# blitzcode/cpp-11-ray-trace-march-framework

Hardware: AMD Instinct MI355X
Metric: Msamples/s at 1920x1080x4spp Cornell-Box+killeroo (higher is better)
Workload: dtype f32; 1 GPU; scenes[1, 8]_1920x1080x4; width=1920, height=1080, spp=4, kernel=0, parallelism=tile-shard x1

## Files before the change

cpp-11-ray-trace-march-framework_amd/__init__.py:

```python
import ctypes
import os

import numpy as np

HERE = os.path.dirname(os.path.abspath(__file__))
KERNEL_SOURCES = ("csrc/rt_kernels.hip", "csrc/rt_walk.h", "csrc/rt_kparams.h", "csrc/rt_plan.hip",
                  "csrc/rt_scene.h", "csrc/rt_tracer.hip", "csrc/rt_grid_build.hip", "csrc/rt_device.h",
                  "csrc/rt_internal.h", "csrc/rt_box_words.h", "csrc/rt_fref_slots.h", "csrc/Makefile",
                  "../include/rt_tracer.h")


def kernel_source_hash():
    import hashlib
    h = hashlib.sha256()
    for rel in KERNEL_SOURCES:
        with open(os.path.normpath(os.path.join(HERE, rel)), "rb") as fh:
            h.update(fh.read())
    return h.hexdigest()[:16]
REPO = os.path.dirname(HERE)
SCENE_DIR = os.path.join(REPO, "data", "scenes")
MESH_DATA_DIR = os.path.join(REPO, "data", "meshes")

RT_TRI_MOLLER_TRUMBORE, RT_TRI_BARYCENTRIC = 0, 1
RT_KERNEL_AUTO, RT_KERNEL_LANES, RT_KERNEL_PIXEL_LOOP, RT_KERNEL_COMPACT = 0, 1, 2, 3
RT_KERNEL_KIND_MASK = 0x07
RT_KERNEL_FLAG_WIDE_HEAVY = 0x200
RT_KERNEL_FLAG_EXHAUSTIVE = 0x8000
RT_KERNEL_FLAG_WAVE_CLOCK = 0x400000
RT_KERNEL_FLAG_OVERLAP = 0x800000
RT_KERNEL_BUDGET_SHIFT = 24
RT_KERNEL_BUDGET_MASK = 0x7F000000
RT_KERNEL_COMPACT_REFILL_SHIFT = RT_KERNEL_BUDGET_SHIFT
RT_ISECT_GRID = 0
RT_ISECT_BRUTE_FORCE = 1
RT_ISECT_RAY_MARCH = 2
SHARD_TILE = 16

TRACER_SYMBOLS = [
    "rt_get_device_count", "rt_scene_create", "rt_scene_destroy", "rt_scene_device_bytes",
    "rt_render_tiles", "rt_render_frame_device", "rt_shard_elems", "rt_render_shard_device",
    "rt_unshard_device", "rt_last_kernel_ms", "rt_trace_samples", "rt_debug_primitives",
# ... 840 lines not shown
```

cpp-11-ray-trace-march-framework_amd/csrc/rt_kernels.hip:

```cpp


#include <hip/hip_runtime.h>

#include <cstddef>
#include <cstdint>

#include "rt_walk.h"

namespace rtk {
namespace {

__device__ __forceinline__ uint32_t xcd_band_block(uint32_t b, uint32_t nb, uint32_t chunk)
{
    if (chunk == 0u)
    {
        const uint32_t q = nb / kXcds, r = nb % kXcds;
        const uint32_t x = b % kXcds, i = b / kXcds;
        return x < r ? x * (q + 1u) + i : r * (q + 1u) + (x - r) * q + i;
    }
    const uint32_t full = nb / (kXcds * chunk) * (kXcds * chunk);
    if (b >= full) return b;
    const uint32_t x = b % kXcds, i = b / kXcds;
    const uint32_t row = (i / chunk) * kXcds + x;
    return row * chunk + i % chunk;
// ... 770 lines not shown
}

__global__ void __launch_bounds__(kWG) k_unshard(const uint32_t *g, uint32_t *out, uint32_t W, uint32_t H,
                                                 uint32_t tiles_x, uint32_t nranks, uint64_t shard_elems)
{
    const uint32_t x = blockIdx.x * 64 + (threadIdx.x & 63u);
    const uint32_t y = blockIdx.y * 4 + (threadIdx.x >> 6);
    if (x >= W || y >= H) return;
    const uint32_t ty = y / kTile, rot = nranks > 1u ? (kShardRot * ty) % tiles_x : 0u;
    const uint32_t tr = x / kTile + rot;
    const uint32_t t = ty * tiles_x + (tr >= tiles_x ? tr - tiles_x : tr);
    const uint32_t r = t % nranks, k = t / nranks;
    out[size_t(y) * W + x] = g[r * shard_elems + size_t(k) * kTilePix + (y % kTile) * kTile + (x % kTile)];
}

__global__ void __launch_bounds__(kWG) k_frame_tables(float *ndc, float2 *smp, TabParams T)
{
    const uint32_t i = blockIdx.x * kWG + threadIdx.x;
    const uint32_t nx = T.W * T.spp, n = (T.W + T.H) * T.spp;
    if (i < T.spp) smp[i] = make_float2(T.smp[2 * i], T.smp[2 * i + 1]);
    if (i >= n) return;
    if (i < nx)
    {
        const uint32_t x = i / T.spp, k = i - x * T.spp;
        ndc[i] = rtd::cam_x(x, T.smp[2 * k], T.W, T.fx);
    }
    else
    {
        const uint32_t j = i - nx, y = j / T.spp, k = j - y * T.spp;
        ndc[i] = rtd::cam_y(y, T.smp[2 * k + 1], T.H, T.fx, T.aspect);
    }
}

__global__ void __launch_bounds__(kWG) k_origin_pre(const float4 *refs, float4 *frefs, uint32_t n, float ox,
                                                    float oy, float oz)
{
    const uint32_t k = blockIdx.x * blockDim.x + threadIdx.x;
    if (k >= n) return;
    const float4 r0 = refs[3 * size_t(k)], r1 = refs[3 * size_t(k) + 1], r2 = refs[3 * size_t(k) + 2];
    const rtd::FRec f = rtd::make_frec(ox, oy, oz, r0.x, r0.y, r0.z, r0.w, r1.x, r1.y, r1.z, r1.w, r2.x);
    frefs[4 * size_t(k) + 0] = f.r0;
    frefs[4 * size_t(k) + 1] = f.r1;
    frefs[4 * size_t(k) + 2] = f.r2;
    frefs[4 * size_t(k) + 3] = f.r3;
}

__global__ void __launch_bounds__(kWG) k_rcp_check(unsigned long long *bad)
{
    const uint64_t n = 1ull << 32;
    for (uint64_t i = uint64_t(blockIdx.x) * blockDim.x + threadIdx.x; i < n; i += uint64_t(gridDim.x) * blockDim.x)
    {
        const uint32_t b = uint32_t(i);
        const uint32_t ex = (b >> 23) & 255u;
        if (ex == 255u || (b & 0x7FFFFFFFu) == 0u) continue;
        const float x = __uint_as_float(b);
        if (__float_as_uint(rtd::rcp_nr(x)) != __float_as_uint(1.0f / x)) atomicAdd(&bad[ex], 1ull);
    }
}

__global__ void __launch_bounds__(kWG) k_gamma_check(unsigned long long *bad)
{
    for (uint32_t b = blockIdx.x * blockDim.x + threadIdx.x; b <= 0x7F800000u; b += gridDim.x * blockDim.x)
    {
        const float x = __uint_as_float(b);
        if (rtd::pack_channel(rtd::gamma_fast(x)) != rtd::pack_channel(rtd::gamma_half(x))) atomicAdd(bad, 1ull);
        if (b == 0x7F800000u) break;
    }
}

__global__ void __launch_bounds__(kWG) k_primitives(int kind, const float *in, uint32_t n, float *out)
{
    const uint32_t i = blockIdx.x * blockDim.x + threadIdx.x;
    if (i >= n) return;
    if (kind == 0)
    {
        const float *a = in + 18 * i;
        float *o = out + 8 * i;
// ... 192 lines not shown
```

cpp-11-ray-trace-march-framework_amd/csrc/rt_kparams.h:

```cpp
#pragma once
#include <hip/hip_runtime.h>

#include <cstdint>

#include "../../include/rt_tracer.h"

namespace rtk {

constexpr uint32_t kTile = 16;
constexpr uint32_t kTilePix = kTile * kTile;
constexpr uint32_t kWG = 256;
constexpr uint32_t kWavesPerWG = kWG / 64u;
constexpr uint32_t kFrefPad = 2u * kWavesPerWG;
constexpr size_t fref_buffer_bytes(uint32_t nrefs) { return (size_t(nrefs ? nrefs : 1u) + kFrefPad) * 64u; }
constexpr int kVarWaveGate = 2;
constexpr int kVarSkipRun = 4;
constexpr int kVarDistSkip = 8;
constexpr int kVarBrute = 64;
constexpr int kVarMarch = 128;
constexpr int kVarExhaustive = 256;
constexpr int kVarOriginPre = 512;
constexpr int kVarFastRcp = 2048;
constexpr int kVarPackedRem = 4096;
constexpr int kVarXcdBands = 8192;
constexpr int kVarWaveClock = 32768;
constexpr int kVarUniform = 65536;
constexpr int kVarWideHeavy = 524288;
constexpr int kVarWideFused = 1048576;
constexpr int kVarWideG4 = 2097152;
constexpr int kVarLdsSplit = 4194304;
constexpr int kVarAutoCore = kVarWaveGate | kVarDistSkip | kVarOriginPre | kVarXcdBands | kVarUniform;
constexpr int kVarAuto = kVarAutoCore | kVarFastRcp | kVarPackedRem | kVarSkipRun;
constexpr int kVarWide = kVarWaveGate | kVarDistSkip | kVarOriginPre | kVarFastRcp | kVarPackedRem | kVarXcdBands;
constexpr int kVarCompactBox = kVarWide | kVarSkipRun;
constexpr uint32_t kMarchSteps = 128;
constexpr uint32_t kDistBlock = 32;
constexpr uint32_t kCompactRefill = 48;

struct HfPlan { uint32_t cnt_hi, cnt_lo, maxc, cnt_w; unsigned long long sum; unsigned long long sum_full; uint32_t cnt_l, pad; };

struct KParams
{
    float m[9];
    float fov_xs, aspect;
    float org[3];
    uint32_t W, H, spp, spp_shift;
    float inv_spp;
    const float2 *smp;
    const float *ndcx;
    const float *ndcy;
    float bmin[3], bmax[3];
    float cw, icw;
    int dim[3];
    int dxdz;
    uint32_t max_steps;
    const uint32_t *off;
    const uint32_t *cellw;
    const uint32_t *cellwo;
    uint32_t oct_stride;
    const uint32_t *cellwb;
    uint32_t box_stride;
    const float4 *refs;
    const float4 *frefs;
    const float4 *shade;
    const float4 *face_n;
    const float4 *tri_mt;
    const float4 *tri_dist;
    const float4 *dist_blk;
    uint32_t ndist_blk;
    float scene_scale;
    float smin[3], smax[3];
    uint32_t ntris;
    uint32_t tri_test;
    uint32_t isect;
    uint32_t rx0, ry0, rw, rh;
    uint32_t tiles_x;
    uint32_t rank, nranks;
    uint32_t wg_per_tile;
    uint32_t xcd_chunk;
    uint32_t vblocks;
    uint64_t *wave_clk;
    const uint32_t *tile_order;
    uint32_t hf_front;
    uint32_t hf_ver;
    uint32_t hf_measure;
    uint32_t hf_floor;
    const uint32_t *hf_mark_in;
    uint32_t *hf_mark_out;
    const uint32_t *hf_list_in;
    uint32_t *hf_list_out;
    const HfPlan *hf_plan_in;
    HfPlan *hf_plan_out;
    uint32_t *hf_cost;
    uint32_t *hf_ticket;
    uint32_t wh_on, wh_wgs, wh_refresh, wh_g;
    uint32_t wh_floor, wh_alpha16;
// ... 47 lines not shown
constexpr int kHfCtxs = 16;
constexpr uint32_t kHfPlanPer = 8;

#ifndef RT_SHARD_ROT
#define RT_SHARD_ROT 3
#endif
constexpr uint32_t kShardRot = RT_SHARD_ROT;

__host__ __device__ __forceinline__ void shard_tile_xy(uint32_t k, uint32_t rank, uint32_t nranks, uint32_t tiles_x,
                                                       uint32_t& tx, uint32_t& ty)
{
    const uint32_t t = rank + k * nranks;
    ty = t / tiles_x;
    tx = t - ty * tiles_x;
    if (nranks > 1u)
    {
        const uint32_t r = (kShardRot * ty) % tiles_x;
        tx = tx >= r ? tx - r : tx + tiles_x - r;
    }
}

using kfn_t = void (*)(KParams);
using kbfn_t = void (*)(KBatch);
using kcfn_t = void (*)(KParams, uint32_t, uint32_t);
using knfn_t = void (*)(KParams, uint32_t);
kfn_t lanes_kernel(int tri, int var);
kfn_t lanes_w64_kernel(int var);
kfn_t wide_kernel(uint32_t g, bool lds);
kfn_t pixel_loop_kernel(int tri, int var);
kcfn_t compact_kernel(int tri, int var);
kbfn_t batch_kernel(int var, bool w64, bool o8 = false);
knfn_t trace_records_kernel();
knfn_t record_fixup_kernel();
using origin_pre_fn = void (*)(const float4 *, float4 *, uint32_t, float, float, float);
using unshard_fn = void (*)(const uint32_t *, uint32_t *, uint32_t, uint32_t, uint32_t, uint32_t, uint64_t);
using check_fn = void (*)(unsigned long long *);
using primitives_fn = void (*)(int, const float *, uint32_t, float *);
origin_pre_fn origin_pre_kernel();
using tables_fn = void (*)(float *, float2 *, TabParams);
tables_fn frame_tables_kernel();
unshard_fn unshard_kernel();
check_fn rcp_check_kernel();
check_fn gamma_check_kernel();
primitives_fn primitives_kernel();

}
```

cpp-11-ray-trace-march-framework_amd/csrc/rt_scene.h:

```cpp
#pragma once
#include <hip/hip_runtime.h>

#include <cstdint>
#include <memory>
#include <mutex>
#include <string>
#include <vector>

#include "../../include/rt_tracer.h"
#include "rt_fref_slots.h"
#include "rt_internal.h"
#include "rt_kparams.h"

#define RT_HIP(expr)                                                                      \
    do {                                                                                  \
        hipError_t e_ = (expr);                                                           \
        if (e_ != hipSuccess)                                                             \
            return rt_internal_fail(RT_E_HIP, std::string(#expr) + ": " + hipGetErrorString(e_)); \
    } while (0)

namespace rtk {

struct EvHolder
{
// ... 31 lines not shown
    bool fence = false;
    hipEvent_t fence_ev = nullptr;
    hipStream_t fence_st = nullptr;
    uint64_t used = 0;
    uint64_t cam = 0;
};

}

constexpr uint32_t kTimeRing = 64;
constexpr uint32_t kTimeEvery = 8;
constexpr uint32_t kMaxBands = 64;
constexpr uint32_t kTileBands = 8;

struct rt_scene
{
    int device = 0;
    std::mutex mtx;
    uint32_t dims[3] = { 0, 0, 0 };
    float bmin[3], bmax[3], cw = 0, icw = 0;
    uint32_t ncells = 0, nrefs = 0, ntris = 0, max_cell_refs = 0;
    uint32_t *d_off = nullptr, *d_cellw = nullptr, *d_cellwo = nullptr, oct_stride = 0;
    uint32_t *d_cellwb = nullptr, box_stride = 0;
    float4 *d_refs = nullptr, *d_shade = nullptr, *d_facen = nullptr;
    float4 *d_trimt = nullptr, *d_tridist = nullptr, *d_distblk = nullptr;
    uint32_t ndist_blk = 0;
    float scene_scale = 0.0f;
    float vmin[3] = { 0, 0, 0 }, vmax[3] = { 0, 0, 0 };
    uint64_t device_bytes = 0;
    uint32_t compact_wgs = 2048;
    bool rcp_safe = false;
    bool pack_ok = false;
    float4 *d_frefs[2] = { nullptr, nullptr };
    rtk::FrefSlots fref;
    uint64_t *d_clk = nullptr;
    size_t clk_cap = 0;
    uint32_t clk_items = 0;
    rtk::HfCtx hf[rtk::kHfCtxs];
    uint32_t *h_wh_cnt = nullptr;
    uint32_t *d_wh_cnt = nullptr;
    uint64_t hf_clock = 0;
    uint64_t hf_evictions = 0;
    uint64_t batch_launches = 0;
    uint64_t batch_fallbacks = 0;
    uint32_t hf_floor = 100000;
    uint32_t hf_min_blocks = 4096;
    uint32_t hf_front_div = 8;
    uint32_t hf_front_max = 1024;
    uint32_t hf_shift = 2;
    uint32_t hf_pos16 = 16;
    uint32_t wh_floor = 100000;
    uint32_t wh_alpha16 = 32;
    uint32_t wh_alpha16_n2 = 16;
    uint32_t wh_alpha16_n4 = 28;
    uint32_t wh_alpha16_n8 = 40;
    uint32_t wh_auto_refs = 128;
    uint32_t wg64 = 1;
    uint32_t wg64_min_blocks = 8192;
    uint32_t wg64_batch_min_blocks = 0;
    uint32_t wg64_max_refs = 1024;
    uint32_t wh_lds = 0x8;
    uint32_t wh_beta16 = 24;
    uint32_t wg64_o8 = 0x2;
    uint32_t wg64_wide = 0xA;
    uint32_t plan_delay = 0;
    uint32_t hf_follow = 1;
// ... 59 lines not shown
```

cpp-11-ray-trace-march-framework_amd/csrc/rt_tracer.hip:

```cpp

#include <hip/hip_runtime.h>
#include <hip/hip_ext.h>

#include <algorithm>
#include <cmath>
#include <cstddef>
#include <chrono>
#include <cstdio>
#include <cstdlib>
#include <cstring>
#include <memory>
#include <mutex>
#include <string>
#include <vector>

#include "../../include/rt_tracer.h"
#include "rt_device.h"
#include "rt_internal.h"
#include "rt_box_words.h"
#include "rt_scene.h"

using namespace rtk;

namespace {
// ... 301 lines not shown
    const float (*c)[4] = reinterpret_cast<const float (*)[4]>(f->cam);
    for (int r = 0; r < 3; r++)
        for (int k = 0; k < 3; k++) P.m[3 * r + k] = c[r][k];
    P.fov_xs = fov_xs_of(f);
    P.aspect = float(f->width) / float(f->height);
    P.ndcx = s->d_ndc;
    P.ndcy = s->d_ndc + size_t(s->ndc_w) * s->ndc_spp;
    for (int k = 0; k < 3; k++)
        P.org[k] = 0.0f * c[0][k] + 0.0f * c[1][k] + 0.0f * c[2][k] + c[3][k];
    P.W = f->width;
    P.H = f->height;
    P.spp = std::max(1u, f->spp);
    P.spp_shift = is_pow2(P.spp) ? log2u(P.spp) : 0;
    P.inv_spp = is_pow2(P.spp) ? 1.0f / float(P.spp) : 0.0f;
    P.smp = s->d_smp;
    for (int a = 0; a < 3; a++)
    {
        P.bmin[a] = s->bmin[a];
        P.bmax[a] = s->bmax[a];
        P.dim[a] = int(s->dims[a]);
    }
    P.cw = s->cw;
    P.icw = s->icw;
    P.dxdz = int(s->dims[0] * s->dims[2]);
    P.max_steps = s->dims[0] + s->dims[1] + s->dims[2] + 3;
    P.off = s->d_off;
    P.cellw = s->d_cellw;
    P.cellwo = s->d_cellwo ? s->d_cellwo : s->d_cellw;
    P.oct_stride = s->d_cellwo ? s->oct_stride : 0u;
    P.cellwb = s->d_cellwb;
    P.box_stride = s->box_stride;
    P.refs = s->d_refs;
    P.frefs = s->d_frefs[0];
    P.shade = s->d_shade;
    P.face_n = s->d_facen;
    P.tri_mt = s->d_trimt;
    P.tri_dist = s->d_tridist;
    P.dist_blk = s->d_distblk;
    P.ndist_blk = s->ndist_blk;
    P.scene_scale = s->scene_scale;
    for (int a = 0; a < 3; a++)
    {
        P.smin[a] = s->vmin[a];
        P.smax[a] = s->vmax[a];
    }
    P.ntris = s->ntris;
    P.tri_test = f->tri_test;
    P.isect = f->intersector;
}

bool use_lanes(const rt_frame *f, uint32_t spp)
{
    if ((f->kernel & RT_KERNEL_KIND_MASK) == RT_KERNEL_PIXEL_LOOP) return false;
    return is_pow2(spp) && spp <= 64;
}

uint32_t env_tunable(const char *name, uint32_t dflt)
{
    const char *e = std::getenv(name);
    return e && *e ? uint32_t(std::strtoul(e, nullptr, 0)) : dflt;
}

bool fref_overlap_ok(const rt_scene *s, const float org[3])
{
    uint32_t ob[3];
    rtk::fref_bits(org, ob);
    return rtk::fref_overlap_ok(s->fref, ob);
}

int ensure_origin_terms(rt_scene *s, KParams& P, hipStream_t st, uint32_t busy, uint32_t *used)
{
    bool compute = false;
    uint32_t ob[3];
    rtk::fref_bits(P.org, ob);
    const int b = rtk::fref_slot_for_launch(s->fref, ob, busy, &compute);
    if (b < 0) return fail(RT_E_INVALID, "internal: no free per-origin record buffer");
    if (compute)
    {
        if (s->nrefs)
            hipLaunchKernelGGL(origin_pre_kernel(), dim3((s->nrefs + kWG - 1) / kWG), dim3(kWG), 0, st, s->d_refs,
                               s->d_frefs[b], s->nrefs, P.org[0], P.org[1], P.org[2]);
        RT_HIP(hipGetLastError());
        rtk::fref_computed(s->fref, b, ob);
    }
    P.frefs = s->d_frefs[b];
    *used |= 1u << b;
    return RT_OK;
}

bool auto_wide(const rt_scene *s, const KParams& P)
{
    return P.nranks >= 2u && s->max_cell_refs >= s->wh_auto_refs;
}

int launch_render(rt_scene *s, const rt_frame *f, KParams& P, uint32_t n_local_tiles, hipStream_t st,
                  bool order_streams = true)
{
    if (n_local_tiles == 0) return RT_OK;
    const bool lanes = use_lanes(f, P.spp);
    P.wg_per_tile = lanes ? (kTilePix * P.spp) / kWG : 1;
    if (P.wg_per_tile == 0) P.wg_per_tile = 1;
    const uint64_t blocks = uint64_t(n_local_tiles) * P.wg_per_tile;
    if (blocks > 0x3FFFFFFFull) return fail(RT_E_INVALID, "frame too large for one launch");
    const uint32_t kind = f->kernel & RT_KERNEL_KIND_MASK;
    const bool bary = P.tri_test == RT_TRI_BARYCENTRIC;
    const bool grid_mt = P.isect == RT_ISECT_GRID && !bary;
    hipStreamCaptureStatus cap = hipStreamCaptureStatusNone;
    RT_HIP(hipStreamIsCapturing(st, &cap));
    bool overlap = false;
    if (order_streams && cap == hipStreamCaptureStatusNone && (f->kernel & RT_KERNEL_FLAG_OVERLAP) && s->ev_recorded &&
        st != s->last_stream &&
        kind == RT_KERNEL_AUTO && lanes && grid_mt && !(f->kernel & (RT_KERNEL_FLAG_WAVE_CLOCK | RT_KERNEL_FLAG_WIDE_HEAVY)) &&
        !auto_wide(s, P) && P.spp <= 64u && !s->tab_dirty)
    {
        overlap = fref_overlap_ok(s, P.org);
        const int v = kVarAutoCore | (s->rcp_safe ? kVarFastRcp : 0) | (auto_runs(s) ? kVarPackedRem | kVarSkipRun : 0);
        if (overlap && blocks >= s->hf_min_blocks)
        {
// ... 472 lines not shown
    const uint32_t nr = g.cell_offsets[nc];
    if (nr && !g.cell_tris) return fail(RT_E_INVALID, "cell_tris is NULL");
    for (uint32_t k = 0; k < nr; k++)
        if (g.cell_tris[k] >= d->num_triangles) return fail(RT_E_INVALID, "cell_tris index out of range");
    for (uint32_t i = 0; i < d->num_triangles; i++)
    {
        const rt_triangle& t = d->triangles[i];
        if (t.v0 >= d->num_vertices || t.v1 >= d->num_vertices || t.v2 >= d->num_vertices)
            return fail(RT_E_INVALID, "triangle vertex index out of range");
    }
    int ncus = 0;
    if (int rc = rt_internal_use_device(device, &ncus)) return rc;

    std::unique_ptr<rt_scene> s(new rt_scene());
    s->device = device;
    s->compact_wgs = 8u * uint32_t(std::max(1, ncus));
    s->hf_floor = env_tunable("RT_HF_FLOOR", s->hf_floor);
    s->hf_min_blocks = env_tunable("RT_HF_MIN_BLOCKS", s->hf_min_blocks);
    s->hf_shift = std::min(env_tunable("RT_HF_SHIFT", s->hf_shift), 8u);
    s->hf_pos16 = std::min(env_tunable("RT_HF_POS16", s->hf_pos16), 64u);
    s->wg64 = env_tunable("RT_WG64", s->wg64);
    s->wh_floor = env_tunable("RT_WH_FLOOR", s->wh_floor);
    s->wh_alpha16 = env_tunable("RT_WH_ALPHA16", s->wh_alpha16);
    s->wh_alpha16_n2 = env_tunable("RT_WH_ALPHA16_N2", s->wh_alpha16_n2);
    s->wh_alpha16_n4 = env_tunable("RT_WH_ALPHA16_N4", s->wh_alpha16_n4);
    s->wh_alpha16_n8 = env_tunable("RT_WH_ALPHA16_N8", s->wh_alpha16_n8);
    s->wh_auto_refs = env_tunable("RT_WH_AUTO_REFS", s->wh_auto_refs);
    s->wg64_max_refs = env_tunable("RT_WG64_MAX_REFS", s->wg64_max_refs);
    s->wg64_wide = env_tunable("RT_WG64_WIDE", s->wg64_wide);
    s->wg64_o8 = env_tunable("RT_WG64_O8", s->wg64_o8);
    s->wh_lds = env_tunable("RT_WH_LDS", s->wh_lds);
    s->wh_beta16 = env_tunable("RT_WH_BETA16", s->wh_beta16);
    s->hf_follow = env_tunable("RT_HF_FOLLOW", s->hf_follow);
    for (int a = 0; a < 3; a++)
    {
        s->dims[a] = g.dims[a];
        s->bmin[a] = g.aabb_min[a];
        s->bmax[a] = g.aabb_max[a];
    }
    s->cw = g.cell_wdh;
    s->icw = g.inv_cell_wdh;
    s->ncells = nc;
    s->nrefs = nr;
    s->ntris = d->num_triangles;

    std::vector<float4> refs(size_t(std::max(nr, 1u)) * 3);
    double det_bound = 0.0;
    for (uint32_t k = 0; k < nr; k++)
    {
        const uint32_t ti = g.cell_tris[k];
        const rt_triangle& t = d->triangles[ti];
        const float *p0 = d->vertices[t.v0].p, *p1 = d->vertices[t.v1].p, *p2 = d->vertices[t.v2].p;
        const float e1[3] = { p1[0] - p0[0], p1[1] - p0[1], p1[2] - p0[2] };
        const float e2[3] = { p2[0] - p0[0], p2[1] - p0[1], p2[2] - p0[2] };
        float idf;
        std::memcpy(&idf, &ti, 4);
        refs[3 * size_t(k) + 0] = make_float4(p0[0], p0[1], p0[2], e1[0]);
        refs[3 * size_t(k) + 1] = make_float4(e1[1], e1[2], e2[0], e2[1]);
        refs[3 * size_t(k) + 2] = make_float4(e2[2], idf, 0.0f, 0.0f);
        const double b = (std::fabs(double(e1[0])) + std::fabs(double(e1[1])) + std::fabs(double(e1[2]))) *
                         (std::fabs(double(e2[0])) + std::fabs(double(e2[1])) + std::fabs(double(e2[2])));
        det_bound = (b > det_bound || b != b) ? b : det_bound;
    }
    s->rcp_safe = det_bound == det_bound && det_bound < 0x1p120;
    s->pack_ok = g.dims[0] <= 512 && g.dims[1] <= 512 && g.dims[2] <= 512;
    std::vector<float4> shade(size_t(d->num_triangles) * 3), facen(d->num_triangles);
// ... 67 lines not shown
                    for (int iz = 0; iz < int(dzs); iz++)
                        for (int ix = 0; ix < int(dxs); ix++)
                        {
                            const int x = sx > 0 ? int(dxs) - 1 - ix : ix;
                            const int y = sy > 0 ? int(dys) - 1 - iy : iy;
                            const int z = sz > 0 ? int(dzs) - 1 - iz : iz;
                            const uint32_t c = uint32_t(x) + uint32_t(z) * dxs + uint32_t(y) * dxs * dzs;
                            if (g.cell_offsets[c + 1] != g.cell_offsets[c]) { D[c] = 0; continue; }
                            uint32_t m = kInf;
                            for (int n = 1; n < 8; n++)
                                m = std::min(m, at(x + ((n & 1) ? sx : 0), y + ((n & 2) ? sy : 0), z + ((n & 4) ? sz : 0)));
                            D[c] = std::min(kInf, m + 1);
                        }
                for (uint32_t c = 0; c < nc; c++)
                    cellwo[size_t(o) * nc + c] = (cellw[c] & 2047u) ? cellw[c] : (D[c] << 11);
            }
        }
        if (nr < (1u << 20) && uint64_t(nc) * 24u * 4u <= kBoxWordsMaxBytes)
        {
            s->box_words = rtbox::build_box_words(g.cell_offsets, g.dims, cellwb);
            if (!s->box_words) cellwb.clear();
        }
    }
    for (uint32_t c = 0; c < nc; c++)
        s->max_cell_refs = std::max(s->max_cell_refs, g.cell_offsets[c + 1] - g.cell_offsets[c]);

    const size_t nfrefs = rtk::fref_buffer_bytes(nr) / sizeof(float4);
    RT_HIP(hipMalloc(&s->d_off, sizeof(uint32_t) * (nc + 1)));
    RT_HIP(hipMalloc(&s->d_refs, sizeof(float4) * refs.size()));
    RT_HIP(hipMalloc(&s->d_frefs[0], sizeof(float4) * nfrefs));
    RT_HIP(hipMalloc(&s->d_frefs[1], sizeof(float4) * nfrefs));
    RT_HIP(hipMemset(s->d_frefs[0], 0, sizeof(float4) * nfrefs));
    RT_HIP(hipMemset(s->d_frefs[1], 0, sizeof(float4) * nfrefs));
    RT_HIP(hipMalloc(&s->d_shade, sizeof(float4) * shade.size()));
    RT_HIP(hipMalloc(&s->d_facen, sizeof(float4) * facen.size()));
    RT_HIP(hipMemcpy(s->d_off, g.cell_offsets, sizeof(uint32_t) * (nc + 1), hipMemcpyHostToDevice));
    RT_HIP(hipMemcpy(s->d_refs, refs.data(), sizeof(float4) * refs.size(), hipMemcpyHostToDevice));
    RT_HIP(hipMemcpy(s->d_shade, shade.data(), sizeof(float4) * shade.size(), hipMemcpyHostToDevice));
    RT_HIP(hipMemcpy(s->d_facen, facen.data(), sizeof(float4) * facen.size(), hipMemcpyHostToDevice));
    std::vector<float4> distblk;
    {
        const uint32_t nt = d->num_triangles;
        float mn[3] = { rtd::kFltMax, rtd::kFltMax, rtd::kFltMax }, mx[3] = { -rtd::kFltMax, -rtd::kFltMax, -rtd::kFltMax };
        float scale = 0.0f;
        for (uint32_t i = 0; i < d->num_vertices; i++)
            for (int a = 0; a < 3; a++)
            {
                mn[a] = std::min(mn[a], d->vertices[i].p[a]);
                mx[a] = std::max(mx[a], d->vertices[i].p[a]);
                scale = std::max(scale, std::fabs(d->vertices[i].p[a]));
            }
        std::vector<std::pair<uint64_t, uint32_t>> order(nt);
        for (uint32_t i = 0; i < nt; i++)
        {
            const rt_triangle& t = d->triangles[i];
            uint64_t code = 0;
            uint32_t q[3];
            for (int a = 0; a < 3; a++)
            {
                const double c = (double(d->vertices[t.v0].p[a]) + d->vertices[t.v1].p[a] + d->vertices[t.v2].p[a]) / 3.0;
                const double ext = double(mx[a]) - double(mn[a]);
                const double f = ext > 0.0 ? (c - mn[a]) / ext : 0.0;
                q[a] = uint32_t(std::min(1023.0, std::max(0.0, f * 1024.0)));
            }
            for (int bit = 9; bit >= 0; bit--)
                for (int a = 0; a < 3; a++) code = (code << 1) | ((q[a] >> bit) & 1u);
// ... 21 lines not shown
            distblk[2 * b + 1] = make_float4(bmx[0], bmx[1], bmx[2], 0.0f);
        }
        s->scene_scale = scale;
        for (int a = 0; a < 3; a++)
        {
            s->vmin[a] = mn[a];
            s->vmax[a] = mx[a];
        }
    }
    RT_HIP(hipMalloc(&s->d_distblk, sizeof(float4) * std::max<size_t>(1, distblk.size())));
    RT_HIP(hipMemcpy(s->d_distblk, distblk.data(), sizeof(float4) * distblk.size(), hipMemcpyHostToDevice));
    RT_HIP(hipMalloc(&s->d_trimt, sizeof(float4) * trimt.size()));
    RT_HIP(hipMalloc(&s->d_tridist, sizeof(float4) * tridist.size()));
    RT_HIP(hipMemcpy(s->d_trimt, trimt.data(), sizeof(float4) * trimt.size(), hipMemcpyHostToDevice));
    RT_HIP(hipMemcpy(s->d_tridist, tridist.data(), sizeof(float4) * tridist.size(), hipMemcpyHostToDevice));
    if (packable)
    {
        RT_HIP(hipMalloc(&s->d_cellw, sizeof(uint32_t) * nc));
        RT_HIP(hipMemcpy(s->d_cellw, cellw.data(), sizeof(uint32_t) * nc, hipMemcpyHostToDevice));
        if (!cellwo.empty())
        {
            RT_HIP(hipMalloc(&s->d_cellwo, sizeof(uint32_t) * cellwo.size()));
            RT_HIP(hipMemcpy(s->d_cellwo, cellwo.data(), sizeof(uint32_t) * cellwo.size(), hipMemcpyHostToDevice));
            s->oct_stride = nc;
        }
        if (!cellwb.empty())
        {
            RT_HIP(hipMalloc(&s->d_cellwb, sizeof(uint32_t) * cellwb.size()));
            RT_HIP(hipMemcpy(s->d_cellwb, cellwb.data(), sizeof(uint32_t) * cellwb.size(), hipMemcpyHostToDevice));
            s->box_stride = nc;
        }
    }
    s->device_bytes = sizeof(uint32_t) * (nc + 1) +
                      sizeof(float4) * (refs.size() + 2 * nfrefs + shade.size() + facen.size() + trimt.size() +
                                        tridist.size() + distblk.size()) +
                      sizeof(uint32_t) * (cellw.size() + cellwo.size() + cellwb.size());
    RT_HIP(hipStreamCreateWithFlags(&s->stream, hipStreamNonBlocking));
    if (int rc = new_event(s->ev_own, s->ev_order_flags)) return rc;
    for (rtk::EvRef& e : s->ev_done)
        if (int rc = new_event(e, s->ev_time_flags)) return rc;
    s->ev_last = s->ev_own;
    RT_HIP(hipStreamCreateWithFlags(&s->plan_st, hipStreamNonBlocking));
    RT_HIP(hipEventCreateWithFlags(&s->kt0[0], s->ev_time_flags));
    if (int rc = new_event(s->kt1[0], s->ev_time_flags)) return rc;
    RT_HIP(hipHostMalloc(&s->h_wh_cnt, sizeof(uint32_t) * 2 * kHfCtxs, hipHostMallocMapped | hipHostMallocCoherent));
    std::memset(s->h_wh_cnt, 0, sizeof(uint32_t) * 2 * kHfCtxs);
    {
        void *dev = nullptr;
        RT_HIP(hipHostGetDevicePointer(&dev, s->h_wh_cnt, 0));
        s->d_wh_cnt = static_cast<uint32_t *>(dev);
    }
    s->ndc_cap = size_t(4096 + 4096) * 16u;
    RT_HIP(hipMalloc(&s->d_ndc, s->ndc_cap * sizeof(float)));
    s->smp_cap = 64u;
    RT_HIP(hipMalloc(&s->d_smp, sizeof(float2) * s->smp_cap));
    RT_HIP(hipHostMalloc(&s->h_smp_pinned, sizeof(float2) * s->smp_cap));
    if (int rc = hf_alloc(&s->hf[0], kHfPreBlocks)) return rc;

    *out = s.release();
    return RT_OK;
}

int rt_scene_destroy(rt_scene *s)
{
    if (!s) return RT_OK;
    {
        std::lock_guard<std::mutex> lk(s->mtx);
        (void)hipSetDevice(s->device);
        if (s->stream) (void)hipStreamSynchronize(s->stream);
        if (s->last_stream && s->ev_recorded) (void)hipEventSynchronize(s->ev_last->ev);
        if (s->ev_prev) (void)hipEventSynchronize(s->ev_prev->ev);
        if (s->plan_st) (void)hipStreamSynchronize(s->plan_st);
        if (s->side) (void)hipStreamSynchronize(s->side);
        (void)hipFree(s->d_off);
        (void)hipFree(s->d_refs);
        (void)hipFree(s->d_frefs[0]);
        (void)hipFree(s->d_frefs[1]);
        (void)hipFree(s->d_shade);
        (void)hipFree(s->d_facen);
        (void)hipFree(s->d_cellw);
        (void)hipFree(s->d_cellwo);
        (void)hipFree(s->d_cellwb);
        (void)hipFree(s->d_trimt);
        (void)hipFree(s->d_tridist);
        (void)hipFree(s->d_distblk);
        (void)hipFree(s->d_clk);
        for (HfCtx& h : s->hf)
        {
            (void)hipFree(h.mem);
            if (h.pend_ev) (void)hipEventDestroy(h.pend_ev);
            if (h.fence_ev) (void)hipEventDestroy(h.fence_ev);
        }
        if (s->h_wh_cnt) (void)hipHostFree(s->h_wh_cnt);
        if (s->side) (void)hipStreamDestroy(s->side);
        if (s->plan_st) (void)hipStreamDestroy(s->plan_st);
        if (s->ev_fork) (void)hipEventDestroy(s->ev_fork);
        if (s->ev_join) (void)hipEventDestroy(s->ev_join);
        (void)hipFree(s->d_smp);
        (void)hipFree(s->d_ndc);
        (void)hipFree(s->d_frame);
        if (s->h_smp_pinned) (void)hipHostFree(s->h_smp_pinned);
        if (s->h_frame) (void)hipHostFree(s->h_frame);
        s->ev_own.reset();
        for (rtk::EvRef& e : s->ev_done) e.reset();
        s->ev_last.reset();
        s->ev_prev.reset();
        for (hipEvent_t e : s->band_ev) if (e) (void)hipEventDestroy(e);
        for (hipEvent_t e : s->kt0) if (e) (void)hipEventDestroy(e);
        for (rtk::EvRef& e : s->kt1) e.reset();
        for (hipEvent_t e : s->tile_ev) if (e) (void)hipEventDestroy(e);
// ... 678 lines not shown
```

cpp-11-ray-trace-march-framework_amd/csrc/rt_walk.h:

```cpp
#pragma once
#include <hip/hip_runtime.h>

#include <cstddef>

#include "rt_device.h"
#include "rt_kparams.h"

namespace rtk {
namespace {

__device__ __forceinline__ uint32_t compact_bits(uint32_t v)
{
    v &= 0x55u;
    v = (v | (v >> 1)) & 0x33u;
    v = (v | (v >> 2)) & 0x0Fu;
    return v;
}

__device__ __forceinline__ void wave_lds_sync()
{
    __builtin_amdgcn_fence(__ATOMIC_RELEASE, "workgroup");
    __builtin_amdgcn_wave_barrier();
    __builtin_amdgcn_fence(__ATOMIC_ACQUIRE, "workgroup");
}

__device__ __forceinline__ void lds_barrier()
{
    asm volatile("s_waitcnt lgkmcnt(0)\n\ts_barrier" ::: "memory");
}

__device__ __forceinline__ float2 *lds_red_tk()
{
    __shared__ float2 r[2 * kWavesPerWG * 64];
    return r;
}
__device__ __forceinline__ float2 *lds_red_uv()
{
    __shared__ float2 r[2 * kWavesPerWG * 64];
    return r;
// ... 96 lines not shown
        const float4 *rp = P.frefs + size_t(k) * 4u;
        const float4 r0 = rp[0], r1 = rp[1], r2 = rp[2];
        float inv, pu;
        const bool ok1 = rtd::mt_rec_first<F>(ra, rc, rtd::f2v{r0.x, r0.y}, rtd::f2v{r0.z, r0.w},
                                              rtd::f2v{r1.x, r1.y}, rtd::f2v{r1.z, r1.w},
                                              rtd::f2v{r2.x, r2.y}, inv, pu);
        if (__any(ok1))
        {
            const float2 r3 = *reinterpret_cast<const float2 *>(rp + 3);
            float pv, pt;
            const bool h = ok1 & rtd::mt_rec_second(ra, rc, rtd::f2v{r2.z, r2.w}, r3.x, r3.y, inv, pu, pv, pt);
            const bool take = h & (pt < tb);
            tb = take ? pt : tb;
            u = take ? pu : u;
            v = take ? pv : v;
            tri = take ? k : tri;
        }
    }
}

template <bool STATS, int TRI, int VAR>
__device__ __forceinline__ bool test_cell(const KParams& P, float ox, float oy, float oz, float dx, float dy,
                                          float dz, uint32_t kb, uint32_t ke, float nct_ax, float& t,
                                          float& u, float& v, uint32_t& tri, uint32_t& tests, uint32_t& lpar)
{
    constexpr bool PRE = (VAR & kVarOriginPre) != 0 && TRI == RT_TRI_MOLLER_TRUMBORE;
    constexpr bool F = (VAR & kVarFastRcp) != 0;
    constexpr bool SPLIT = (VAR & kVarLdsSplit) != 0;
    static_assert(!SPLIT || (PRE && !STATS), "the LDS tier runs AUTO's record test");
    (void)lpar;
    bool split = false;
    if constexpr (SPLIT) split = __any(ke - kb >= kLdsSplitMin);
    const uint32_t first = split ? __builtin_amdgcn_readfirstlane(threadIdx.x >> 6) : 0u, step = split ? kWavesPerWG : 1u;
    const rtd::f2v ra = {dx, dy}, rc = {dy, dz};
    const float tb0 = t < nct_ax ? t : nct_ax;
    float tb = tb0;
    bool uniform_done = false;
    if constexpr ((VAR & kVarUniform) != 0 && PRE)
    {
        const uint32_t kb0 = __builtin_amdgcn_readfirstlane(kb), ke0 = __builtin_amdgcn_readfirstlane(ke);
        uint32_t diff = (kb ^ kb0) | (ke ^ ke0);
        asm volatile("" : "+v"(diff));
        if (wave_all(diff == 0u))
        {
            if constexpr ((VAR & kVarWaveClock) != 0)
                if (first_active_lane()) wave_counters()[0] += ke0 - kb0;
            cvf4 *crefs = (cvf4 *)P.frefs;
            const uint32_t kfirst = kb0 + (SPLIT ? first : 0u), kstep = SPLIT ? step : 1u;
            if (!SPLIT || kfirst < ke0)
            {
                auto rec_k = [&](cvf4 *p, uint32_t ahead) {
                    uint64_t d = uint64_t(p) - uint64_t(crefs);
                    asm("" : "+s"(d));
                    return uint32_t(d >> 6) + ahead;
                };
                auto test_rec = [&](const vf4 r0, const vf4 r1, const vf4 r2, const vf4 r3, auto pos) {
                    if (STATS) tests++;
                    float inv, cu;
                    const bool ok1 = rtd::mt_rec_first<F>(ra, rc, rtd::f2v{r0.x, r0.y}, rtd::f2v{r0.z, r0.w},
                                                          rtd::f2v{r1.x, r1.y}, rtd::f2v{r1.z, r1.w},
                                                          rtd::f2v{r2.x, r2.y}, inv, cu);
                    if (__any(ok1))
                    {
                        float cv, ct;
                        const bool hit = ok1 & rtd::mt_rec_second(ra, rc, rtd::f2v{r2.z, r2.w}, r3.x, r3.y, inv, cu,
                                                                  cv, ct);
                        const bool take = hit & (ct < tb);
                        tb = take ? ct : tb;
                        u = take ? cu : u;
                        v = take ? cv : v;
                        const uint32_t k = pos();
                        tri = take ? k : tri;
                    }
                };
                cvf4 *np = crefs + size_t(kfirst) * 4u;
                if constexpr (!SPLIT)
                {
                    const uint32_t n = ke0 - kb0;
                    cvf4 *const endp = np + size_t(n >> 1) * 8u;
                    vf16 a, b;
                    asm volatile("s_load_dwordx16 %0, %1, 0x0" : "=&s"(a) : "s"(np));
                    asm volatile("s_waitcnt lgkmcnt(0)" : "+s"(a));
                    if (np != endp)
                        do
                        {
                            asm volatile("s_load_dwordx16 %0, %1, 0x40" : "=&s"(b) : "s"(np));
                            test_rec(vf4{a[0], a[1], a[2], a[3]}, vf4{a[4], a[5], a[6], a[7]},
                                     vf4{a[8], a[9], a[10], a[11]}, vf4{a[12], a[13], a[14], a[15]},
                                     [&] { return rec_k(np, 0u); });
                            asm volatile("s_waitcnt lgkmcnt(0)" : "+s"(b));
                            asm volatile("s_load_dwordx16 %0, %1, 0x80" : "=&s"(a) : "s"(np));
                            test_rec(vf4{b[0], b[1], b[2], b[3]}, vf4{b[4], b[5], b[6], b[7]},
                                     vf4{b[8], b[9], b[10], b[11]}, vf4{b[12], b[13], b[14], b[15]},
                                     [&] { return rec_k(np, 1u); });
                            asm volatile("s_waitcnt lgkmcnt(0)" : "+s"(a));
                            np += 8;
                            asm volatile("" : "+s"(np));
                        } while (np != endp);
                    if (n & 1u)
                        test_rec(vf4{a[0], a[1], a[2], a[3]}, vf4{a[4], a[5], a[6], a[7]},
                                 vf4{a[8], a[9], a[10], a[11]}, vf4{a[12], a[13], a[14], a[15]},
                                 [&] { return rec_k(np, 0u); });
                }
                else
                {
                vf4 a0 = np[0], a1 = np[1], a2 = np[2], a3 = np[3];
                for (uint32_t k = kfirst;; k += 2u * kstep)
                {
                    vf4 b0, b1, b2, b3;
                    const bool more1 = k + kstep < ke0;
                    if (more1)
                    {
                        np = crefs + size_t(k + kstep) * 4u;
                        b0 = np[0];
                        b1 = np[1];
                        b2 = np[2];
                        b3 = np[3];
                    }
                    test_rec(a0, a1, a2, a3, [&] { return k; });
                    if (!more1) break;
                    const bool more2 = k + 2u * kstep < ke0;
                    if (more2)
                    {
                        np = crefs + size_t(k + 2u * kstep) * 4u;
                        a0 = np[0];
                        a1 = np[1];
                        a2 = np[2];
                        a3 = np[3];
                    }
                    test_rec(b0, b1, b2, b3, [&] { return k + kstep; });
                    if (!more2) break;
                }
                }
            }
            uniform_done = true;
// ... 751 lines not shown
```

Baseline: 33480 Msamples/s.

## Add conservative per-triangle gate records to skip full intersection tests

Precomputes, per triangle reference, a compact 32-byte gate record (half-normal-like planes plus a rounded-up error bound, built in double precision) alongside the origin-relative fref records. In the non-split scalar-load triangle loop for lists of at least eight triangles, waves first test two gates per 64-byte scalar load and only fetch and run the full Moller-Trumbore record test when some lane is not rejected. The aim is to cut scalar memory traffic and ALU per cell list. The cost is extra gate computation and buffers, plus a serialized load-and-wait for each surviving record, which loses the previous prefetch overlap when few triangles are rejected.

Measured after the change: 35180 Msamples/s, median of 6. 1.05x the previous value.

```diff
diff --git a/cpp-11-ray-trace-march-framework_amd/__init__.py b/cpp-11-ray-trace-march-framework_amd/__init__.py
--- a/cpp-11-ray-trace-march-framework_amd/__init__.py
+++ b/cpp-11-ray-trace-march-framework_amd/__init__.py
@@ -6,7 +6,7 @@
 HERE = os.path.dirname(os.path.abspath(__file__))
 KERNEL_SOURCES = ("csrc/rt_kernels.hip", "csrc/rt_walk.h", "csrc/rt_kparams.h", "csrc/rt_plan.hip",
                   "csrc/rt_scene.h", "csrc/rt_tracer.hip", "csrc/rt_grid_build.hip", "csrc/rt_device.h",
-                  "csrc/rt_internal.h", "csrc/rt_box_words.h", "csrc/rt_fref_slots.h", "csrc/Makefile",
+                  "csrc/rt_internal.h", "csrc/rt_box_words.h", "csrc/rt_fref_slots.h", "csrc/rt_record_gate.h", "csrc/Makefile",
                   "../include/rt_tracer.h")
 
 
diff --git a/cpp-11-ray-trace-march-framework_amd/csrc/rt_kernels.hip b/cpp-11-ray-trace-march-framework_amd/csrc/rt_kernels.hip
--- a/cpp-11-ray-trace-march-framework_amd/csrc/rt_kernels.hip
+++ b/cpp-11-ray-trace-march-framework_amd/csrc/rt_kernels.hip
@@ -826,8 +826,8 @@
     }
 }
 
-__global__ void __launch_bounds__(kWG) k_origin_pre(const float4 *refs, float4 *frefs, uint32_t n, float ox,
-                                                    float oy, float oz)
+__global__ void __launch_bounds__(kWG) k_origin_pre(const float4 *refs, float4 *frefs, float4 *gates, uint32_t n,
+                                                    float ox, float oy, float oz)
 {
     const uint32_t k = blockIdx.x * blockDim.x + threadIdx.x;
     if (k >= n) return;
@@ -837,6 +837,13 @@
     frefs[4 * size_t(k) + 1] = f.r1;
     frefs[4 * size_t(k) + 2] = f.r2;
     frefs[4 * size_t(k) + 3] = f.r3;
+    if (gates)
+    {
+        float g[kGateFloats];
+        make_gate(r0.w, r1.x, r1.y, r1.z, r1.w, r2.x, f.r0.y, f.r0.w, f.r1.y, g);
+        gates[2 * size_t(k) + 0] = make_float4(g[0], g[1], g[2], g[3]);
+        gates[2 * size_t(k) + 1] = make_float4(g[4], g[5], g[6], g[7]);
+    }
 }
 
 __global__ void __launch_bounds__(kWG) k_rcp_check(unsigned long long *bad)
diff --git a/cpp-11-ray-trace-march-framework_amd/csrc/rt_kparams.h b/cpp-11-ray-trace-march-framework_amd/csrc/rt_kparams.h
--- a/cpp-11-ray-trace-march-framework_amd/csrc/rt_kparams.h
+++ b/cpp-11-ray-trace-march-framework_amd/csrc/rt_kparams.h
@@ -13,6 +13,11 @@
 constexpr uint32_t kWavesPerWG = kWG / 64u;
 constexpr uint32_t kFrefPad = 2u * kWavesPerWG;
 constexpr size_t fref_buffer_bytes(uint32_t nrefs) { return (size_t(nrefs ? nrefs : 1u) + kFrefPad) * 64u; }
+constexpr size_t gate_buffer_bytes(uint32_t nrefs) { return (size_t(nrefs ? nrefs : 1u) + kFrefPad) * 32u; }
+#ifndef RT_GATE_MIN_LIST
+#define RT_GATE_MIN_LIST 8
+#endif
+constexpr uint32_t kGateMinList = RT_GATE_MIN_LIST;
 constexpr int kVarWaveGate = 2;
 constexpr int kVarSkipRun = 4;
 constexpr int kVarDistSkip = 8;
@@ -62,6 +67,7 @@
     uint32_t box_stride;
     const float4 *refs;
     const float4 *frefs;
+    const float4 *gates;
     const float4 *shade;
     const float4 *face_n;
     const float4 *tri_mt;
@@ -175,7 +181,7 @@
 kbfn_t batch_kernel(int var, bool w64, bool o8 = false);
 knfn_t trace_records_kernel();
 knfn_t record_fixup_kernel();
-using origin_pre_fn = void (*)(const float4 *, float4 *, uint32_t, float, float, float);
+using origin_pre_fn = void (*)(const float4 *, float4 *, float4 *, uint32_t, float, float, float);
 using unshard_fn = void (*)(const uint32_t *, uint32_t *, uint32_t, uint32_t, uint32_t, uint32_t, uint64_t);
 using check_fn = void (*)(unsigned long long *);
 using primitives_fn = void (*)(int, const float *, uint32_t, float *);
diff --git a/cpp-11-ray-trace-march-framework_amd/csrc/rt_record_gate.h b/cpp-11-ray-trace-march-framework_amd/csrc/rt_record_gate.h
--- /dev/null
+++ b/cpp-11-ray-trace-march-framework_amd/csrc/rt_record_gate.h
@@ -0,0 +1,74 @@
+#pragma once
+#include <cstdint>
+
+#if defined(__HIPCC__)
+#define RT_GATE_HD __host__ __device__ __forceinline__
+#else
+#define RT_GATE_HD inline
+#endif
+
+namespace rtk {
+
+constexpr uint32_t kGateFloats = 8;
+constexpr double kGateDmax = 1.0001;
+constexpr double kGateU = 1.0 / 16777216.0;
+constexpr double kGateMaxIn = 1099511627776.0;
+
+RT_GATE_HD double gate_abs(double x) { return x < 0.0 ? -x : x; }
+
+RT_GATE_HD float gate_round_up(double x)
+{
+    if (!(x < 3.0e38)) return __builtin_inff();
+    float e = float(x);
+    if (double(e) < x)
+    {
+        uint32_t b;
+        __builtin_memcpy(&b, &e, 4);
+        b += 1u;
+        __builtin_memcpy(&e, &b, 4);
+    }
+    return e;
+}
+
+RT_GATE_HD void make_gate(float e1x, float e1y, float e1z, float e2x, float e2y, float e2z, float tx, float ty,
+                          float tz, float g[kGateFloats])
+{
+    const double a1[3] = { e1x, e1y, e1z }, a2[3] = { e2x, e2y, e2z }, at[3] = { tx, ty, tz };
+    bool big = false;
+    for (int i = 0; i < 3; i++)
+        big = big || !(gate_abs(a1[i]) <= kGateMaxIn) || !(gate_abs(a2[i]) <= kGateMaxIn) ||
+              !(gate_abs(at[i]) <= kGateMaxIn);
+    const double nh[3] = { 0.5 * (a2[1] * a1[2] - a2[2] * a1[1]), 0.5 * (a2[2] * a1[0] - a2[0] * a1[2]),
+                           0.5 * (a2[0] * a1[1] - a2[1] * a1[0]) };
+    const double nz[3] = { (a2[1] * at[2] - a2[2] * at[1]) - nh[0], (a2[2] * at[0] - a2[0] * at[2]) - nh[1],
+                           (a2[0] * at[1] - a2[1] * at[0]) - nh[2] };
+    const float fz[3] = { float(nz[0]), float(nz[1]), float(nz[2]) }, fh[3] = { float(nh[0]), float(nh[1]), float(nh[2]) };
+    const double s[3] = { gate_abs(a2[1]) + gate_abs(a2[2]), gate_abs(a2[0]) + gate_abs(a2[2]),
+                          gate_abs(a2[0]) + gate_abs(a2[1]) };
+    const double sum_e1 = gate_abs(a1[0]) * s[0] + gate_abs(a1[1]) * s[1] + gate_abs(a1[2]) * s[2];
+    const double sum_t = gate_abs(at[0]) * s[0] + gate_abs(at[1]) * s[1] + gate_abs(at[2]) * s[2];
+    const double n1z = gate_abs(double(fz[0])) + gate_abs(double(fz[1])) + gate_abs(double(fz[2]));
+    const double n1h = gate_abs(double(fh[0])) + gate_abs(double(fh[1])) + gate_abs(double(fh[2]));
+    const double ud = kGateU * kGateDmax;
+    const double B = 6.0 * ud * sum_t + 1.01 * (6.0 * ud * sum_e1) + 4.0 * ud * n1z + 4.0 * ud * n1h + 6.0 * ud * n1h;
+    const double E = 2.0 * B * (1.0 + 1.0 / 1048576.0) + 0x1p-100;
+    const float Ef = big ? __builtin_inff() : gate_round_up(E);
+    const bool off = !(Ef < __builtin_inff());
+    g[0] = off ? 0.0f : fz[0];
+    g[1] = off ? 0.0f : fh[0];
+    g[2] = off ? 0.0f : fz[1];
+    g[3] = off ? 0.0f : fh[1];
+    g[4] = off ? 0.0f : fz[2];
+    g[5] = off ? 0.0f : fh[2];
+    g[6] = off ? __builtin_inff() : Ef;
+    g[7] = 0.0f;
+}
+
+template <class V2>
+RT_GATE_HD bool gate_rejects(float dx, float dy, float dz, V2 n0, V2 n1, V2 n2, float E)
+{
+    const V2 m = (n0 * dx + n1 * dy) + n2 * dz;
+    return __builtin_fabsf(m.x) > __builtin_fabsf(m.y) + E;
+}
+
+}
diff --git a/cpp-11-ray-trace-march-framework_amd/csrc/rt_scene.h b/cpp-11-ray-trace-march-framework_amd/csrc/rt_scene.h
--- a/cpp-11-ray-trace-march-framework_amd/csrc/rt_scene.h
+++ b/cpp-11-ray-trace-march-framework_amd/csrc/rt_scene.h
@@ -87,6 +87,8 @@
     bool rcp_safe = false;
     bool pack_ok = false;
     float4 *d_frefs[2] = { nullptr, nullptr };
+    float4 *d_gates[2] = { nullptr, nullptr };
+    bool rec_gate = true;
     rtk::FrefSlots fref;
     uint64_t *d_clk = nullptr;
     size_t clk_cap = 0;
diff --git a/cpp-11-ray-trace-march-framework_amd/csrc/rt_tracer.hip b/cpp-11-ray-trace-march-framework_amd/csrc/rt_tracer.hip
--- a/cpp-11-ray-trace-march-framework_amd/csrc/rt_tracer.hip
+++ b/cpp-11-ray-trace-march-framework_amd/csrc/rt_tracer.hip
@@ -357,6 +357,7 @@
     P.box_stride = s->box_stride;
     P.refs = s->d_refs;
     P.frefs = s->d_frefs[0];
+    P.gates = s->rec_gate ? s->d_gates[0] : nullptr;
     P.shade = s->d_shade;
     P.face_n = s->d_facen;
     P.tri_mt = s->d_trimt;
@@ -404,11 +405,13 @@
     {
         if (s->nrefs)
             hipLaunchKernelGGL(origin_pre_kernel(), dim3((s->nrefs + kWG - 1) / kWG), dim3(kWG), 0, st, s->d_refs,
-                               s->d_frefs[b], s->nrefs, P.org[0], P.org[1], P.org[2]);
+                               s->d_frefs[b], s->rec_gate ? s->d_gates[b] : nullptr, s->nrefs, P.org[0], P.org[1],
+                               P.org[2]);
         RT_HIP(hipGetLastError());
         rtk::fref_computed(s->fref, b, ob);
     }
     P.frefs = s->d_frefs[b];
+    P.gates = s->rec_gate ? s->d_gates[b] : nullptr;
     *used |= 1u << b;
     return RT_OK;
 }
@@ -947,6 +950,7 @@
     s->wh_lds = env_tunable("RT_WH_LDS", s->wh_lds);
     s->wh_beta16 = env_tunable("RT_WH_BETA16", s->wh_beta16);
     s->hf_follow = env_tunable("RT_HF_FOLLOW", s->hf_follow);
+    s->rec_gate = env_tunable("RT_REC_GATE", 1u) != 0u;
     for (int a = 0; a < 3; a++)
     {
         s->dims[a] = g.dims[a];
@@ -1080,6 +1084,13 @@
     RT_HIP(hipMalloc(&s->d_frefs[1], sizeof(float4) * nfrefs));
     RT_HIP(hipMemset(s->d_frefs[0], 0, sizeof(float4) * nfrefs));
     RT_HIP(hipMemset(s->d_frefs[1], 0, sizeof(float4) * nfrefs));
+    if (rtk::fref_buffer_bytes(nr) > 0xFFFFFFFFull) s->rec_gate = false;
+    const size_t ngates = rtk::gate_buffer_bytes(nr) / sizeof(float4);
+    for (int b = 0; b < 2; b++)
+    {
+        RT_HIP(hipMalloc(&s->d_gates[b], sizeof(float4) * ngates));
+        RT_HIP(hipMemset(s->d_gates[b], 0, sizeof(float4) * ngates));
+    }
     RT_HIP(hipMalloc(&s->d_shade, sizeof(float4) * shade.size()));
     RT_HIP(hipMalloc(&s->d_facen, sizeof(float4) * facen.size()));
     RT_HIP(hipMemcpy(s->d_off, g.cell_offsets, sizeof(uint32_t) * (nc + 1), hipMemcpyHostToDevice));
@@ -1167,7 +1178,7 @@
         }
     }
     s->device_bytes = sizeof(uint32_t) * (nc + 1) +
-                      sizeof(float4) * (refs.size() + 2 * nfrefs + shade.size() + facen.size() + trimt.size() +
+                      sizeof(float4) * (refs.size() + 2 * nfrefs + 2 * ngates + shade.size() + facen.size() + trimt.size() +
                                         tridist.size() + distblk.size()) +
                       sizeof(uint32_t) * (cellw.size() + cellwo.size() + cellwb.size());
     RT_HIP(hipStreamCreateWithFlags(&s->stream, hipStreamNonBlocking));
@@ -1211,6 +1222,8 @@
         (void)hipFree(s->d_refs);
         (void)hipFree(s->d_frefs[0]);
         (void)hipFree(s->d_frefs[1]);
+        (void)hipFree(s->d_gates[0]);
+        (void)hipFree(s->d_gates[1]);
         (void)hipFree(s->d_shade);
         (void)hipFree(s->d_facen);
         (void)hipFree(s->d_cellw);
diff --git a/cpp-11-ray-trace-march-framework_amd/csrc/rt_walk.h b/cpp-11-ray-trace-march-framework_amd/csrc/rt_walk.h
--- a/cpp-11-ray-trace-march-framework_amd/csrc/rt_walk.h
+++ b/cpp-11-ray-trace-march-framework_amd/csrc/rt_walk.h
@@ -5,6 +5,7 @@
 
 #include "rt_device.h"
 #include "rt_kparams.h"
+#include "rt_record_gate.h"
 
 namespace rtk {
 namespace {
@@ -167,7 +168,7 @@
     bool split = false;
     if constexpr (SPLIT) split = __any(ke - kb >= kLdsSplitMin);
     const uint32_t first = split ? __builtin_amdgcn_readfirstlane(threadIdx.x >> 6) : 0u, step = split ? kWavesPerWG : 1u;
-    const rtd::f2v ra = {dx, dy}, rc = {dy, dz};
+    rtd::f2v ra = {dx, dy}, rc = {dy, dz};
     const float tb0 = t < nct_ax ? t : nct_ax;
     float tb = tb0;
     bool uniform_done = false;
@@ -212,8 +213,73 @@
                 if constexpr (!SPLIT)
                 {
                     const uint32_t n = ke0 - kb0;
+                    vf16 a, b;
+                    cvf4 *const cgates = (cvf4 *)P.gates;
+                    bool gated = false;
+                    if constexpr (!STATS) gated = n >= kGateMinList && cgates != nullptr;
+                    if (gated)
+                    {
+                        cvf4 *gp = cgates + size_t(kb0) * 2u;
+                        uint32_t k = kb0;
+                        const uint32_t kend = kb0 + (n & ~3u);
+                        auto gate_pair = [&](vf16& s, uint32_t ahead, bool two) {
+                            using rtd::f2v;
+                            asm("" : "+v"(ra), "+v"(rc));
+                            const bool ja = gate_rejects(ra.x, ra.y, rc.y, f2v{s[0], s[1]}, f2v{s[2], s[3]},
+                                                         f2v{s[4], s[5]}, s[6]);
+                            const bool jb = gate_rejects(ra.x, ra.y, rc.y, f2v{s[8], s[9]}, f2v{s[10], s[11]},
+                                                         f2v{s[12], s[13]}, s[14]);
+                            const uint64_t ma = __builtin_amdgcn_ballot_w64(!ja);
+                            const uint64_t mb = two ? __builtin_amdgcn_ballot_w64(!jb) : 0ull;
+                            if ((ma | mb) != 0ull)
+                            {
+                                if (ma != 0ull)
+                                {
+                                    const uint32_t ro = (k + ahead) << 6;
+                                    asm volatile("s_load_dwordx16 %0, %1, %2" : "=&s"(s) : "s"(crefs), "s"(ro));
+                                    asm volatile("s_waitcnt lgkmcnt(0)" : "+s"(s));
+                                    test_rec(vf4{s[0], s[1], s[2], s[3]}, vf4{s[4], s[5], s[6], s[7]},
+                                             vf4{s[8], s[9], s[10], s[11]}, vf4{s[12], s[13], s[14], s[15]},
+                                             [&] { return k + ahead; });
+                                }
+                                if (mb != 0ull)
+                                {
+                                    const uint32_t ro = (k + ahead + 1u) << 6;
+                                    asm volatile("s_load_dwordx16 %0, %1, %2" : "=&s"(s) : "s"(crefs), "s"(ro));
+                                    asm volatile("s_waitcnt lgkmcnt(0)" : "+s"(s));
+                                    test_rec(vf4{s[0], s[1], s[2], s[3]}, vf4{s[4], s[5], s[6], s[7]},
+                                             vf4{s[8], s[9], s[10], s[11]}, vf4{s[12], s[13], s[14], s[15]},
+                                             [&] { return k + ahead + 1u; });
+                                }
+                            }
+                        };
+                        asm volatile("s_load_dwordx16 %0, %1, 0x0" : "=&s"(a) : "s"(gp));
+                        asm volatile("s_waitcnt lgkmcnt(0)" : "+s"(a));
+                        if (k != kend)
+                            do
+                            {
+                                asm volatile("s_load_dwordx16 %0, %1, 0x40" : "=&s"(b) : "s"(gp));
+                                gate_pair(a, 0u, true);
+                                asm volatile("s_waitcnt lgkmcnt(0)" : "+s"(b));
+                                asm volatile("s_load_dwordx16 %0, %1, 0x80" : "=&s"(a) : "s"(gp));
+                                gate_pair(b, 2u, true);
+                                asm volatile("s_waitcnt lgkmcnt(0)" : "+s"(a));
+                                gp += 8;
+                                k += 4u;
+                                asm volatile("" : "+s"(gp), "+s"(k));
+                            } while (k != kend);
+                        const uint32_t rem = n & 3u;
+                        if (rem != 0u)
+                        {
+                            asm volatile("s_load_dwordx16 %0, %1, 0x40" : "=&s"(b) : "s"(gp));
+                            gate_pair(a, 0u, rem >= 2u);
+                            asm volatile("s_waitcnt lgkmcnt(0)" : "+s"(b));
+                            if (rem == 3u) gate_pair(b, 2u, false);
+                        }
+                    }
+                    else
+                    {
                     cvf4 *const endp = np + size_t(n >> 1) * 8u;
-                    vf16 a, b;
                     asm volatile("s_load_dwordx16 %0, %1, 0x0" : "=&s"(a) : "s"(np));
                     asm volatile("s_waitcnt lgkmcnt(0)" : "+s"(a));
                     if (np != endp)
@@ -236,6 +302,7 @@
                         test_rec(vf4{a[0], a[1], a[2], a[3]}, vf4{a[4], a[5], a[6], a[7]},
                                  vf4{a[8], a[9], a[10], a[11]}, vf4{a[12], a[13], a[14], a[15]},
                                  [&] { return rec_k(np, 0u); });
+                    }
                 }
                 else
                 {
```
